# HeewoongNoh/DOSTransformer

Measured on NVIDIA B200. Metric: train-step crystals/sec (fwd+bwd), higher is better.
Workload: dtype bf16x3 operands, f32 accumulate

## Files before the change

dostransformer_b200/_lib.py:

```python
from __future__ import annotations

import ctypes as C
import os
from typing import Optional

import torch

_HERE = os.path.dirname(os.path.abspath(__file__))
LIB_PATH = os.environ.get("DOST_B200_LIB") or os.path.join(_HERE, "libdost_b200.so")

F32, F64 = 0, 1
ACT_NONE, ACT_RELU, ACT_LEAKY, ACT_PRELU = 0, 1, 2, 3
KC, MC = 0, 1
PREC_FMA, PREC_BF16X3, PREC_BF16 = 0, 1, 2
PRECISIONS = {"fp32": PREC_FMA, "bf16x3": PREC_BF16X3, "bf16": PREC_BF16}

_lib: Optional[C.CDLL] = None
ABI_VERSION = 15
DEVERR_MESSAGES = {1: "an index (edge_index / batch / system) is outside its table",
                   2: "a crystal has more atoms than the padding length given by the host (max_num_nodes)"}


class Seg(C.Structure):
    _fields_ = [("base", C.c_void_p), ("ld", C.c_longlong), ("idx", C.c_void_p), ("div", C.c_int),
# ... 101 lines not shown
                                 C.c_void_p, C.c_longlong, C.c_void_p, C.c_void_p, C.c_int, C.c_int, C.c_int, C.c_int,
                                 C.c_double, C.c_double, C.c_ulonglong, C.c_void_p]),
    "dost_xattn_bwd_workspace_bytes": (C.c_size_t, [C.c_int, C.c_int, C.c_int, C.c_int]),
    "dost_xattn_bwd": (C.c_int, [C.c_int, C.c_void_p, C.c_void_p, C.c_longlong, C.c_void_p, C.c_void_p, C.c_void_p,
                                 C.c_void_p, C.c_void_p, C.c_void_p, C.c_void_p, C.c_longlong, C.c_void_p, C.c_void_p,
                                 C.c_void_p, C.c_void_p, C.c_int, C.c_int, C.c_int, C.c_int, C.c_longlong, C.c_double,
                                 C.c_double, C.c_ulonglong, C.c_void_p, C.c_size_t, C.c_void_p]),
    "dost_xattn_kv_ext_build": (C.c_int, [C.c_void_p, C.c_void_p, C.c_void_p, C.c_void_p, C.c_longlong, C.c_int, C.c_int, C.c_void_p,
                                          C.c_void_p, C.c_longlong, C.c_void_p]),
    "dost_xattn_kv_ext_split": (C.c_int, [C.c_void_p, C.c_void_p, C.c_void_p, C.c_longlong, C.c_int, C.c_int, C.c_void_p, C.c_void_p,
                                          C.c_void_p]),
    "dost_xattn_kv_pad_split": (C.c_int, [C.c_void_p, C.c_int, C.c_int, C.c_void_p, C.c_void_p, C.c_longlong, C.c_int, C.c_int, C.c_void_p,
                                          C.c_void_p, C.c_void_p]),
    "dost_xattn_softmax_fwd": (C.c_int, [C.c_void_p, C.c_void_p, C.c_void_p, C.c_longlong, C.c_int, C.c_int, C.c_int, C.c_double,
                                         C.c_void_p, C.c_void_p, C.c_longlong, C.c_void_p, C.c_double, C.c_ulonglong, C.c_void_p]),
    "dost_xattn_softmax_bwd": (C.c_int, [C.c_void_p, C.c_void_p, C.c_void_p, C.c_void_p, C.c_void_p, C.c_longlong, C.c_int, C.c_int,
                                         C.c_int, C.c_double, C.c_void_p, C.c_void_p, C.c_longlong, C.c_double, C.c_ulonglong,
                                         C.c_void_p]),
    "dost_softmax_fwd": (C.c_int, [C.c_int, C.c_void_p, C.c_void_p, C.c_void_p, C.c_longlong, C.c_int, C.c_longlong, C.c_double,
                                   C.c_double, C.c_ulonglong, C.c_void_p]),
    "dost_softmax_bwd": (C.c_int, [C.c_int, C.c_void_p, C.c_void_p, C.c_void_p, C.c_longlong, C.c_int, C.c_longlong, C.c_double,
                                   C.c_double, C.c_ulonglong, C.c_void_p]),
    "dost_softmax_fwd_planes": (C.c_int, [C.c_void_p, C.c_void_p, C.c_void_p, C.c_longlong, C.c_int, C.c_longlong, C.c_double,
                                          C.c_double, C.c_ulonglong, C.c_void_p, C.c_void_p, C.c_longlong, C.c_void_p]),
    "dost_softmax_bwd_planes": (C.c_int, [C.c_void_p, C.c_void_p, C.c_void_p, C.c_longlong, C.c_int, C.c_longlong, C.c_double,
                                          C.c_double, C.c_ulonglong, C.c_void_p, C.c_void_p, C.c_longlong, C.c_void_p]),
    "dost_attn_fused_supported": (C.c_int, [C.c_int, C.c_int, C.c_int]),
    "dost_attn_fused_fwd": (C.c_int, [C.c_void_p, C.c_void_p, C.c_longlong, C.c_void_p, C.c_void_p, C.c_longlong, C.c_longlong,
                                      C.c_int, C.c_int, C.c_int, C.c_int, C.c_void_p, C.c_void_p, C.c_void_p, C.c_int, C.c_double,
                                      C.c_void_p, C.c_longlong, C.c_void_p, C.c_void_p, C.c_void_p, C.c_longlong, C.c_int,
                                      C.c_double, C.c_ulonglong, C.c_void_p, C.c_void_p]),
    "dost_softmax_bwd_from_planes": (C.c_int, [C.c_void_p, C.c_void_p, C.c_longlong, C.c_void_p, C.c_longlong, C.c_longlong, C.c_int,
                                               C.c_double, C.c_void_p, C.c_void_p, C.c_longlong, C.c_void_p]),
    "dost_eval_metrics": (C.c_int, [C.c_int, C.c_void_p, C.c_void_p, C.c_int, C.c_int, C.c_int, C.c_void_p, C.c_void_p, C.c_void_p]),
    "dost_adamw_step": (C.c_int, [C.c_int, C.c_void_p, C.c_void_p, C.c_void_p, C.c_void_p, C.c_void_p, C.c_double, C.c_double,
                                  C.c_double, C.c_double, C.c_double, C.c_longlong, C.c_void_p]),
    "dost_loss_fwd": (C.c_int, [C.c_int, C.c_int, C.c_void_p, C.c_void_p, C.c_void_p, C.c_double, C.c_int, C.c_int,
                                C.c_void_p, C.c_void_p, C.c_void_p]),
    "dost_loss_bwd": (C.c_int, [C.c_int, C.c_int, C.c_void_p, C.c_void_p, C.c_void_p, C.c_double, C.c_int, C.c_int,
                                C.c_void_p, C.c_void_p, C.c_void_p, C.c_void_p, C.c_void_p]),
    "dost_collate_ptr": (C.c_int, [C.c_void_p, C.c_longlong, C.c_void_p, C.c_void_p, C.c_longlong, C.c_void_p, C.c_void_p,
                                   C.c_void_p, C.c_void_p, C.c_void_p]),
    "dost_collate_rows": (C.c_int, [C.c_void_p, C.c_void_p, C.c_void_p, C.c_void_p, C.c_longlong, C.c_longlong,
                                    C.c_longlong, C.c_void_p, C.c_void_p]),
    "dost_collate_index": (C.c_int, [C.c_void_p, C.c_longlong, C.c_void_p, C.c_void_p, C.c_void_p, C.c_void_p, C.c_void_p,
                                     C.c_longlong, C.c_longlong, C.c_longlong, C.c_void_p, C.c_void_p, C.c_void_p]),
    "dost_neighbor_count": (C.c_int, [C.c_void_p, C.c_void_p, C.c_void_p, C.c_void_p, C.c_longlong, C.c_double, C.c_int,
                                      C.c_void_p, C.c_void_p]),
    "dost_neighbor_fill": (C.c_int, [C.c_void_p, C.c_void_p, C.c_void_p, C.c_void_p, C.c_longlong, C.c_double, C.c_int,
                                     C.c_void_p, C.c_int, C.c_void_p, C.c_void_p, C.c_void_p, C.c_void_p, C.c_void_p,
                                     C.c_void_p]),
    "dost_knn_select": (C.c_int, [C.c_void_p, C.c_void_p, C.c_void_p, C.c_longlong, C.c_int, C.c_longlong, C.c_double,
                                  C.c_void_p, C.c_void_p, C.c_void_p, C.c_void_p]),
    "dost_gaussian_expand": (C.c_int, [C.c_void_p, C.c_longlong, C.c_double, C.c_double, C.c_int, C.c_double, C.c_void_p,
                                       C.c_void_p]),
}


def _with_seed_offset(args):
    i = args.index(C.c_ulonglong) + 1
    return args[:i] + [C.c_void_p] + args[i:]


for _name in ("dost_xattn_fwd", "dost_xattn_bwd", "dost_xattn_softmax_fwd", "dost_xattn_softmax_bwd", "dost_softmax_fwd",
              "dost_softmax_bwd", "dost_softmax_fwd_planes", "dost_softmax_bwd_planes", "dost_attn_fused_fwd"):
    _res, _args = _SIGNATURES[_name]
# ... 105 lines not shown
```

dostransformer_b200/csrc/tc_ptx.cuh:

```cuda
#pragma once
#include <cuda.h>
#include <cuda_bf16.h>
#include <cstdint>

namespace dost {
namespace ptx {

__device__ __forceinline__ uint32_t smem_u32(const void* p) { return static_cast<uint32_t>(__cvta_generic_to_shared(p)); }
__device__ __forceinline__ void mbar_init(uint32_t bar, uint32_t count) {
  asm volatile("mbarrier.init.shared::cta.b64 [%0], %1;" ::"r"(bar), "r"(count) : "memory");
}
__device__ __forceinline__ void mbar_arrive(uint32_t bar) {
  asm volatile("mbarrier.arrive.shared::cta.b64 _, [%0];" ::"r"(bar) : "memory");
}
__device__ __forceinline__ void mbar_expect_tx(uint32_t bar, uint32_t bytes) {
  asm volatile("mbarrier.arrive.expect_tx.shared::cta.b64 _, [%0], %1;" ::"r"(bar), "r"(bytes) : "memory");
}
__device__ __forceinline__ void mbar_wait(uint32_t bar, uint32_t parity) {
  asm volatile(
      "{\n\t"
      ".reg .pred P1;\n\t"
      "WAIT_LOOP:\n\t"
      "mbarrier.try_wait.parity.shared::cta.b64 P1, [%0], %1, %2;\n\t"
      "@P1 bra WAIT_DONE;\n\t"
// ... 47 lines not shown
}
__device__ __forceinline__ uint32_t cluster_ctarank() {
  uint32_t r;
  asm volatile("mov.u32 %0, %%cluster_ctarank;" : "=r"(r));
  return r;
}
__device__ __forceinline__ void cluster_sync_all() {
  asm volatile("barrier.cluster.arrive.release.aligned;" ::: "memory");
  asm volatile("barrier.cluster.wait.acquire.aligned;" ::: "memory");
}
__device__ __forceinline__ uint32_t mapa_rank(uint32_t addr, uint32_t rank) {
  uint32_t r;
  asm volatile("mapa.shared::cluster.u32 %0, %1, %2;" : "=r"(r) : "r"(addr), "r"(rank));
  return r;
}
__device__ __forceinline__ void mbar_arrive_cluster(uint32_t cluster_bar) {
  asm volatile("mbarrier.arrive.relaxed.cluster.shared::cluster.b64 _, [%0];" ::"r"(cluster_bar) : "memory");
}
__device__ __forceinline__ void umma_commit_2cta(uint32_t bar) {
  asm volatile("tcgen05.commit.cta_group::2.mbarrier::arrive::one.shared::cluster.multicast::cluster.b64 [%0], %1;" ::"r"(bar),
               "h"(static_cast<uint16_t>(3))
               : "memory");
}
__device__ __forceinline__ void umma_f16_2cta(uint32_t tmem_d, uint64_t adesc, uint64_t bdesc, uint32_t idesc, uint32_t accum) {
  asm volatile(
      "{\n\t"
      ".reg .pred p;\n\t"
      "setp.ne.b32 p, %4, 0;\n\t"
      "tcgen05.mma.cta_group::2.kind::f16 [%0], %1, %2, %3, p;\n\t"
      "}" ::"r"(tmem_d),
      "l"(adesc), "l"(bdesc), "r"(idesc), "r"(accum)
      : "memory");
}
__device__ __forceinline__ void tma_load_3d_2cta(uint32_t dst, const CUtensorMap* map, int c0, int c1, int c2, uint32_t cluster_bar) {
  asm volatile(
      "cp.async.bulk.tensor.3d.cta_group::2.shared::cluster.global.mbarrier::complete_tx::bytes [%0], [%1, {%2, %3, %4}], [%5];" ::"r"(
          dst),
      "l"(map), "r"(c0), "r"(c1), "r"(c2), "r"(cluster_bar)
      : "memory");
}

__device__ __forceinline__ void tmem_ld_wait() { asm volatile("tcgen05.wait::ld.sync.aligned;" ::: "memory"); }

__device__ __forceinline__ void tma_load_3d(uint32_t dst, const CUtensorMap* map, int c0, int c1, int c2, uint32_t bar) {
  asm volatile(
      "cp.async.bulk.tensor.3d.shared::cluster.global.mbarrier::complete_tx::bytes [%0], [%1, {%2, %3, %4}], [%5];" ::"r"(dst),
      "l"(map), "r"(c0), "r"(c1), "r"(c2), "r"(bar)
      : "memory");
}

__device__ __forceinline__ uint32_t make_idesc(int m, int n, bool a_mn, bool b_mn) {
  return (1u << 4) | (1u << 7) | (1u << 10) | ((a_mn ? 1u : 0u) << 15) | ((b_mn ? 1u : 0u) << 16) |
         (static_cast<uint32_t>(n >> 3) << 17) | (static_cast<uint32_t>(m >> 4) << 24);
}

__device__ __forceinline__ void sts128(uint32_t addr, uint32_t a, uint32_t b, uint32_t c, uint32_t d) {
  asm volatile("st.shared.v4.b32 [%0], {%1, %2, %3, %4};" ::"r"(addr), "r"(a), "r"(b), "r"(c), "r"(d) : "memory");
}
__device__ __forceinline__ float4 lds128(uint32_t addr) {
  float4 v;
  asm volatile("ld.shared.v4.f32 {%0, %1, %2, %3}, [%4];" : "=f"(v.x), "=f"(v.y), "=f"(v.z), "=f"(v.w) : "r"(addr) : "memory");
  return v;
}


__device__ __forceinline__ void tma_store_3d(const CUtensorMap* map, uint32_t src, int c0, int c1, int c2) {
// ... 43 lines not shown
```

dostransformer_b200/ops.py:

```python
from __future__ import annotations

import ctypes as C
import math
from contextlib import nullcontext
import os
from dataclasses import dataclass, field
from typing import List, Optional, Sequence, Tuple

import torch

from . import _lib as L

NUM_SMS = 148

_PRECISION = L.PREC_FMA


def set_precision(name: str) -> None:
    global _PRECISION
    _PRECISION = L.PRECISIONS[name]


def get_precision() -> int:
    return _PRECISION
# ... 402 lines not shown
    if residual is not None:
        g.residual, g.ld_res = residual.data_ptr(), (ld_res if ld_res is not None else _ld(residual))
    if out is not None:
        g.out = out.data_ptr()
        g.ldc = ldc if ldc is not None else _ld(out)
    g.accumulate = 1 if accumulate else 0
    g.batch, g.a_bstride, g.b_bstride, g.c_bstride, g.res_bstride = batch, a_bstride, b_bstride, c_bstride, res_bstride
    g.b_rowoff = b_rowoff.data_ptr() if b_rowoff is not None else None
    g.c_rowoff = c_rowoff.data_ptr() if c_rowoff is not None else None
    g.c_rowlim = c_rowlim.data_ptr() if c_rowlim is not None else None
    if out_planes is not None:
        g.out_hi = out_planes.hi.data_ptr()
        g.out_lo = out_planes.lo.data_ptr() if out_planes.lo is not None else None
        g.ld_op = out_planes.ld
    g.split_k = split_k
    g.precision = _PRECISION if prec is None else prec
    g.colsum = colsum_out.data_ptr() if colsum_out is not None else None
    if out_gate is not None:
        g.out_gate, g.ld_gate = out_gate.data_ptr(), out_gate.stride(0)
    if dact_gate is not None:
        g.dact_gate, g.ld_gate, g.dact_slope = dact_gate.data_ptr(), dact_gate.stride(0), dact_slope
    lib = L.lib()
    ws, nb = None, 0
    if split_k > 1 or colsum_out is not None:
        nb = lib.dost_gemm_bf16_workspace_bytes(C.byref(g))
        ws = _ws(nb, b.hi.device)
    L.check(lib.dost_gemm_bf16(C.byref(g), L.p(ws), nb, L.stream()), "gemm_bf16")


def gate_bits_ok(M: int, N: int) -> bool:
    return M >= 32 and N % 32 == 0 and os.environ.get("DOST_GEMM_TMA_EPI", "1") != "0" and not L.switch("DOST_NO_FFN_GATE")


def tc_active(t: torch.Tensor) -> bool:
    return _PRECISION != L.PREC_FMA and t.dtype == torch.float32


def _with_lo() -> bool:
    return _PRECISION != L.PREC_BF16


def ln_fwd_planes(x2d: torch.Tensor, gamma, beta, slope=None, *, want_y: bool = False, want_planes: bool = True,
                  gather_add=None):
    M, W = x2d.shape
    ga = ia = gb = ib = None
    ldg = 0
    if gather_add is not None:
        ga, ia, gb, ib = gather_add
        ldg = _ld(ga)
        assert _ld(gb) == ldg
    dev = x2d.device
    y = torch.empty(M, W, dtype=torch.float32, device=dev) if want_y else None
    pl = empty_planes(M, W, dev, _with_lo()) if want_planes else None
    stats = torch.empty(M, 2, dtype=torch.float32, device=dev)
    L.check(L.lib().dost_ln_fwd_planes(L.p(x2d), _ld(x2d), L.p(ga), L.p(ia), L.p(gb), L.p(ib), ldg, L.p(gamma), L.p(beta),
                                       L.p(slope), L.p(y),
                                       L.p(pl.hi) if pl else None, L.p(pl.lo) if (pl and pl.lo is not None) else None,
                                       pl.ld if pl else 0, L.p(stats), M, W, L.stream()), "ln_fwd_planes")
    return y, pl, stats


def ln_bwd_planes(dy2d, x2d, stats, gamma, beta, slope=None, *, dres=None, want_dx: bool = True, want_planes: bool = False,
                  want_xsum: bool = False):
    M, W = x2d.shape
    dev = x2d.device
    dx = torch.empty(M, W, dtype=torch.float32, device=dev) if want_dx else None
# ... 21 lines not shown
    L.check(lib.dost_colsum_planes(L.p(pl.hi), L.p(pl.lo), pl.ld, pl.rows, pl.cols, L.p(out), L.p(ws), nb, L.stream()),
            "colsum_planes")
    return out


def _split_for(M_out: int, N_out: int, K_red: int) -> int:
    bn = 64 if N_out <= 64 else (128 if N_out <= 128 else 256)
    tiles = math.ceil(M_out / 128) * math.ceil(N_out / bn)
    want = max(1, (2 * NUM_SMS) // tiles)
    return int(max(1, min(want, math.ceil(K_red / 512), 256)))


def _planes_save(pl: Planes):
    return [pl.hi, pl.lo]


def _planes_load(hi, lo, rows, cols) -> Planes:
    return Planes(hi, lo, rows, cols)


class _FFNBlock(torch.autograd.Function):

    @staticmethod
    def forward(ctx, y_nd, ln_w, ln_b, w1, b1, w2, b2):
        H = y_nd.shape[-1]
        y = y_nd.reshape(-1, H)
        if y.stride(-1) != 1 or (y.shape[0] > 1 and y.stride(0) != H):
            y = y.contiguous()
        M = y.shape[0]
        F = w1.shape[0]
        dev = y.device
        _, h0p, stats = ln_fwd_planes(y, ln_w, ln_b)
        w1p, w2p = weight_planes(w1), weight_planes(w2)
        h1p = empty_planes(M, F, dev, _with_lo())
        gate = torch.empty(F // 32, M, dtype=torch.int32, device=dev) if (gate_bits_ok(M, F) and any(ctx.needs_input_grad)) else None
        gemm_planes(M=M, N=F, K=H, a=[h0p], a_mode=L.KC, b=w1p, b_mode=L.KC, bias=b1, act=L.ACT_RELU, out_planes=h1p, out_gate=gate)
        out = torch.empty(M, H, dtype=torch.float32, device=dev)
        gemm_planes(M=M, N=H, K=F, a=[h1p], a_mode=L.KC, b=w2p, b_mode=L.KC, bias=b2, residual=y, out=out)
        ctx.save_for_backward(y, stats, ln_w, ln_b, w1, w2, *_planes_save(h0p), *_planes_save(h1p), gate)
        ctx.prec = _PRECISION
        ctx.shape = y_nd.shape
        ctx.emit_grad_planes = bool(getattr(y_nd, "_dost_attn_out", False))
        return out.view(y_nd.shape)

    @staticmethod
    def backward(ctx, d_out_nd):
        y, stats, ln_w, ln_b, w1, w2, h0h, h0l, h1h, h1l, gate = ctx.saved_tensors
        M, H = y.shape
        F = w1.shape[0]
        dev = y.device
        with precision_value(ctx.prec):
            h0p, h1p = _planes_load(h0h, h0l, M, H), _planes_load(h1h, h1l, M, F)
            w1p, w2p = weight_planes(w1), weight_planes(w2)
            dop = getattr(d_out_nd, "_dost_planes", None)
            db2 = getattr(d_out_nd, "_dost_colsum", None)
            d_out = d_out_nd.reshape(M, H)
            if d_out.stride(-1) != 1 or (M > 1 and d_out.stride(0) != H):
                d_out, dop = d_out.contiguous(), None
            if dop is None or db2 is None or dop.rows != M or dop.cols != H or (dop.lo is not None) != _with_lo() or \
                    getattr(d_out_nd, "_dost_planes_version", -1) != d_out_nd._version:
                dop, db2 = split_planes_colsum(d_out)
            dw2 = torch.empty(H, F, dtype=torch.float32, device=dev)
            gemm_planes(M=H, N=F, K=M, a=[dop], a_mode=L.MC, b=h1p, b_mode=L.MC, out=dw2, split_k=_split_for(H, F, M))
            dv1p = empty_planes(M, F, dev, _with_lo())
            db1 = torch.empty(F, dtype=torch.float32, device=dev)
            gemm_planes(M=M, N=F, K=H, a=[dop], a_mode=L.KC, b=w2p, b_mode=L.MC, dact=h1p if gate is None else None,
                        dact_gate=gate, dact_slope=0.0, out_planes=dv1p, colsum_out=db1)
            dw1 = torch.empty(F, H, dtype=torch.float32, device=dev)
            gemm_planes(M=F, N=H, K=M, a=[dv1p], a_mode=L.MC, b=h0p, b_mode=L.MC, out=dw1, split_k=_split_for(F, H, M))
            dh0 = torch.empty(M, H, dtype=torch.float32, device=dev)
            gemm_planes(M=M, N=H, K=F, a=[dv1p], a_mode=L.KC, b=w1p, b_mode=L.MC, out=dh0)
            dy, dyp, dg, db, _, _ = ln_bwd_planes(dh0, y, stats, ln_w, ln_b, dres=d_out, want_planes=ctx.emit_grad_planes)
# ... 1059 lines not shown
```

include/dost.h:

```cpp
#ifndef DOST_H_
#define DOST_H_

#include <stddef.h>
#include <stdint.h>

#ifdef __cplusplus
extern "C" {
#endif

#define DOST_ABI_VERSION 15

enum { DOST_F32 = 0, DOST_F64 = 1 };
enum { DOST_OK = 0, DOST_ERR_ARG = -1, DOST_ERR_LAUNCH = -2, DOST_ERR_WORKSPACE = -3, DOST_ERR_UNSUPPORTED = -4 };
enum { DOST_ACT_NONE = 0, DOST_ACT_RELU = 1, DOST_ACT_LEAKY = 2, DOST_ACT_PRELU = 3 };
enum { DOST_PREC_FMA = 0, DOST_PREC_BF16X3 = 1 , DOST_PREC_BF16 = 2 };
enum { DOST_KC = 0 , DOST_MC = 1  };

typedef void* dost_stream_t;

int dost_abi_version(void);
const char* dost_last_error(void);
long long dost_launch_count(void);
void dost_reset_launch_count(void);

// ... 179 lines not shown
                     double drop_p, unsigned long long seed, dost_stream_t stream);
int dost_softmax_fwd_dseed(int dtype, const void* s, void* p, void* pd, long long rows, int cols, long long ld, double scale,
                           double drop_p, unsigned long long seed, const unsigned long long* seed_offset, dost_stream_t stream);
int dost_softmax_bwd_dseed(int dtype, const void* p, const void* dpd, void* ds, long long rows, int cols, long long ld,
                           double scale, double drop_p, unsigned long long seed, const unsigned long long* seed_offset,
                           dost_stream_t stream);

int dost_softmax_fwd_planes(const float* s, float* p, float* pd, long long rows, int cols, long long ld, double scale,
                            double drop_p, unsigned long long seed, void* hi, void* lo, long long ldp, dost_stream_t stream);
int dost_softmax_bwd_planes(const float* p, const float* dpd, float* ds, long long rows, int cols, long long ld, double scale,
                            double drop_p, unsigned long long seed, void* hi, void* lo, long long ldp, dost_stream_t stream);
int dost_softmax_fwd_planes_dseed(const float* s, float* p, float* pd, long long rows, int cols, long long ld, double scale,
                                  double drop_p, unsigned long long seed, const unsigned long long* seed_offset, void* hi,
                                  void* lo, long long ldp, dost_stream_t stream);
int dost_softmax_bwd_planes_dseed(const float* p, const float* dpd, float* ds, long long rows, int cols, long long ld,
                                  double scale, double drop_p, unsigned long long seed, const unsigned long long* seed_offset,
                                  void* hi, void* lo, long long ldp, dost_stream_t stream);

int dost_attn_fused_supported(int Lq, int H, int max_keys);
int dost_attn_fused_fwd(const void* q_hi, const void* q_lo, long long ld_q, const void* k_hi, const void* k_lo, long long ld_k,
                        long long k_rows, int S, int Lq, int Lk, int H, const int32_t* k_rowoff, const int32_t* k_count,
                        const int32_t* nmax, int max_keys, double scale, const float* residual, long long res_seq_stride,
                        float* out, void* p_hi, void* p_lo, long long ld_p, int precision, double drop_p,
                        unsigned long long seed, float* lse, dost_stream_t stream);
int dost_attn_fused_fwd_dseed(const void* q_hi, const void* q_lo, long long ld_q, const void* k_hi, const void* k_lo,
                              long long ld_k, long long k_rows, int S, int Lq, int Lk, int H, const int32_t* k_rowoff,
                              const int32_t* k_count, const int32_t* nmax, int max_keys, double scale, const float* residual,
                              long long res_seq_stride, float* out, void* p_hi, void* p_lo, long long ld_p, int precision,
                              double drop_p, unsigned long long seed, const unsigned long long* seed_offset, float* lse,
                              dost_stream_t stream);
int dost_softmax_bwd_from_planes(const void* p_hi, const void* p_lo, long long ld_pp, const float* dP, long long ld_dp,
                                 long long rows, int cols, double scale, void* hi, void* lo, long long ldp, dost_stream_t stream);

int dost_loss_fwd(int dtype, int mode, const void* pred_g, const void* pred_s, const void* y, double beta, int B,
                  int T, void* loss, void* saved, dost_stream_t stream);
int dost_loss_bwd(int dtype, int mode, const void* pred_g, const void* pred_s, const void* y, double beta, int B,
                  int T, const void* saved, const void* grad_loss, void* d_pred_g, void* d_pred_s,
                  dost_stream_t stream);

int dost_eval_metrics(int dtype, const void* pred, const void* y, int clamp_pred, int B, int T, void* per_crystal, void* mean,
                      dost_stream_t stream);

int dost_adamw_step(int ntensors, void* const* params, const void* const* grads, void* const* exp_avg,
                    void* const* exp_avg_sq, const long long* numel, double lr, double beta1, double beta2, double eps,
                    double weight_decay, long long step, dost_stream_t stream);

int dost_collate_ptr(const int64_t* ids, long long B, const int64_t* node_ptr_all, const int64_t* edge_ptr_all,
                     long long C, int64_t* node_ptr_out, int64_t* edge_ptr_out, int64_t* nmax_out, int32_t* bad_flag,
                     dost_stream_t stream);
int dost_collate_rows(const void* src, const int64_t* src_ptr_all, const int64_t* ids, const int64_t* out_ptr,
                      long long B, long long rows_out, long long row_bytes, void* dst, dost_stream_t stream);
int dost_collate_index(const int64_t* edge_index_all, long long E_all, const int64_t* node_ptr_all,
                       const int64_t* edge_ptr_all, const int64_t* ids, const int64_t* node_ptr_out,
                       const int64_t* edge_ptr_out, long long B, long long N_out, long long E_out,
                       int64_t* edge_index_out, int64_t* batch_out, dost_stream_t stream);

int dost_neighbor_count(const double* lattice, const double* pos, const int64_t* node_ptr, const int64_t* crystal_of,
                        long long N, double cutoff, int self_interaction, int64_t* count, dost_stream_t stream);
int dost_neighbor_fill(const double* lattice, const double* pos, const int64_t* node_ptr, const int64_t* crystal_of,
                       long long N, double cutoff, int self_interaction, const int64_t* edge_ptr, int local_ids,
                       int64_t* edge_src, int64_t* edge_dst, int64_t* edge_shift, double* edge_vec, double* edge_len,
                       dost_stream_t stream);
int dost_knn_select(const int64_t* edge_ptr, const int64_t* edge_dst, const double* edge_len, long long N, int k,
                    long long pad_idx, double pad_dist, int64_t* out_idx, double* out_dist, int64_t* out_edge,
                    dost_stream_t stream);
int dost_gaussian_expand(const double* dist, long long n, double dmin, double step, int nfilt, double var, float* out,
// ... 7 lines not shown
```

Measured before the change: 21090.

## Fuse FFN forward into a single 2-CTA tcgen05 kernel keeping hidden in TMEM

```diff
diff --git a/dostransformer_b200/_lib.py b/dostransformer_b200/_lib.py
--- a/dostransformer_b200/_lib.py
+++ b/dostransformer_b200/_lib.py
@@ -157,6 +157,11 @@
                                       C.c_double, C.c_ulonglong, C.c_void_p, C.c_void_p]),
     "dost_softmax_bwd_from_planes": (C.c_int, [C.c_void_p, C.c_void_p, C.c_longlong, C.c_void_p, C.c_longlong, C.c_longlong, C.c_int,
                                                C.c_double, C.c_void_p, C.c_void_p, C.c_longlong, C.c_void_p]),
+    "dost_ffn_fused_supported": (C.c_int, [C.c_int, C.c_int, C.c_int]),
+    "dost_ffn_fwd_fused": (C.c_int, [C.c_int, C.c_int, C.c_int, C.c_int, C.c_void_p, C.c_void_p, C.c_longlong, C.c_void_p,
+                                     C.c_void_p, C.c_longlong, C.c_void_p, C.c_void_p, C.c_void_p, C.c_longlong, C.c_void_p,
+                                     C.c_void_p, C.c_longlong, C.c_void_p, C.c_longlong, C.c_void_p, C.c_void_p, C.c_longlong,
+                                     C.c_void_p, C.c_longlong, C.c_void_p]),
     "dost_eval_metrics": (C.c_int, [C.c_int, C.c_void_p, C.c_void_p, C.c_int, C.c_int, C.c_int, C.c_void_p, C.c_void_p, C.c_void_p]),
     "dost_adamw_step": (C.c_int, [C.c_int, C.c_void_p, C.c_void_p, C.c_void_p, C.c_void_p, C.c_void_p, C.c_double, C.c_double,
                                   C.c_double, C.c_double, C.c_double, C.c_longlong, C.c_void_p]),
diff --git a/dostransformer_b200/csrc/ffn_fused.cu b/dostransformer_b200/csrc/ffn_fused.cu
--- /dev/null
+++ b/dostransformer_b200/csrc/ffn_fused.cu
@@ -0,0 +1,491 @@
+#include <cuda.h>
+#include <cuda_bf16.h>
+#include "common.cuh"
+#include "tc_ptx.cuh"
+
+namespace dost {
+namespace ffn {
+
+using namespace ptx;
+
+__device__ __forceinline__ void mbar_arrive_release_cluster(uint32_t cluster_bar) {
+  asm volatile("mbarrier.arrive.release.cluster.shared::cluster.b64 _, [%0];" ::"r"(cluster_bar) : "memory");
+}
+
+constexpr int BM = 128, BK = 64, FC = 128, HD = 256;
+constexpr int kEpiWarps = 8, kThreads = (kEpiWarps + 2) * 32;
+constexpr int kStgBytes = 4096;
+constexpr int kStageRing = 192 * 1024;
+constexpr int kSmemBytes = kStageRing + kEpiWarps * kStgBytes + 1024;
+constexpr int kMaxStages = 8;
+
+struct Maps {
+  CUtensorMap x_hi, x_lo, w1_hi, w1_lo, w2_hi, w2_lo;
+  CUtensorMap out, h_hi, h_lo;
+};
+
+struct Params {
+  int M, F, m_tiles;
+  const float* b1;
+  const float* b2;
+  const float* res; long long ld_res;
+  unsigned int* gate; long long ld_gate;
+  int store_h;
+};
+
+template <int NSPLIT>
+__global__ void __launch_bounds__(kThreads, 1) ffn_fwd_kernel(const __grid_constant__ Maps maps, const Params p) {
+  constexpr bool SPLIT = NSPLIT == 3;
+  constexpr int NP = SPLIT ? 2 : 1;
+  constexpr int XB = BM * BK * 2;
+  constexpr int W1B = (FC / 2) * BK * 2;
+  constexpr int W2B = (HD / 2) * BK * 2;
+  constexpr int A_BYTES = NP * (XB + W1B), B_BYTES = NP * W2B;
+  constexpr int STAGE = A_BYTES;
+  constexpr int NSTAGE = kStageRing / STAGE;
+  static_assert(B_BYTES <= STAGE && NSTAGE >= 2 && NSTAGE <= kMaxStages, "stage ring");
+
+  extern __shared__ __align__(1024) unsigned char smem_raw[];
+  unsigned char* smem = reinterpret_cast<unsigned char*>((reinterpret_cast<uintptr_t>(smem_raw) + 1023) & ~uintptr_t(1023));
+  __shared__ __align__(8) unsigned long long bars[2 * kMaxStages + 6];
+  __shared__ uint32_t tmem_base_s;
+
+  const int warp = threadIdx.x >> 5, lane = threadIdx.x & 31;
+  const uint32_t full0 = smem_u32(&bars[0]), empty0 = smem_u32(&bars[kMaxStages]);
+  const uint32_t acc1f0 = smem_u32(&bars[2 * kMaxStages]);
+  const uint32_t pready0 = smem_u32(&bars[2 * kMaxStages + 2]);
+  const uint32_t acc2f = smem_u32(&bars[2 * kMaxStages + 4]);
+  const uint32_t acc2e = smem_u32(&bars[2 * kMaxStages + 5]);
+  const int NC = p.F / FC;
+  const int rank = (int)cluster_ctarank();
+  const int tile0 = (int)(blockIdx.x >> 1), tile_step = (int)(gridDim.x >> 1);
+
+  if (threadIdx.x == 0) {
+    for (int s = 0; s < NSTAGE; ++s) {
+      mbar_init(full0 + 8 * s, 1);
+      mbar_init(empty0 + 8 * s, 1);
+    }
+    for (int b = 0; b < 2; ++b) {
+      mbar_init(acc1f0 + 8 * b, 1);
+      mbar_init(pready0 + 8 * b, 2 * kEpiWarps);
+    }
+    mbar_init(acc2f, 1);
+    mbar_init(acc2e, 2 * kEpiWarps);
+    fence_barrier_init();
+  }
+  if (warp == kEpiWarps) {
+    asm volatile("tcgen05.alloc.cta_group::2.sync.aligned.shared::cta.b32 [%0], %1;" ::"r"(smem_u32(&tmem_base_s)), "r"(512) : "memory");
+    asm volatile("tcgen05.relinquish_alloc_permit.cta_group::2.sync.aligned;" ::: "memory");
+  }
+  tc_fence_before();
+  __syncthreads();
+  cluster_sync_all();
+  tc_fence_after();
+  const uint32_t tmem_base = tmem_base_s;
+
+  if (warp == kEpiWarps + 1) {
+    if (lane == 0) {
+      int stage = 0;
+      uint32_t phase = 0;
+      auto next = [&]() {
+        if (++stage == NSTAGE) {
+          stage = 0;
+          phase ^= 1;
+        }
+      };
+      for (int tile = tile0; tile < p.m_tiles; tile += tile_step) {
+        const int m0 = tile * 2 * BM + rank * BM;
+        auto begin = [&](int bytes) {
+          mbar_wait(empty0 + 8 * stage, phase ^ 1);
+          if (rank == 0) mbar_expect_tx(full0 + 8 * stage, 2 * bytes);
+          return mapa_rank(full0 + 8 * stage, 0);
+        };
+        auto load_a = [&](int c) {
+          for (int kt = 0; kt < HD / BK; ++kt) {
+            const uint32_t bar = begin(A_BYTES);
+            const uint32_t s = smem_u32(smem + stage * STAGE);
+            const int w1row = c * FC + rank * (FC / 2);
+            tma_load_3d_2cta(s, &maps.x_hi, kt * BK, m0, 0, bar);
+            tma_load_3d_2cta(s + NP * XB, &maps.w1_hi, kt * BK, w1row, 0, bar);
+            if (SPLIT) {
+              tma_load_3d_2cta(s + XB, &maps.x_lo, kt * BK, m0, 0, bar);
+              tma_load_3d_2cta(s + 2 * XB + W1B, &maps.w1_lo, kt * BK, w1row, 0, bar);
+            }
+            next();
+          }
+        };
+        auto load_b = [&](int c) {
+          for (int kt = 0; kt < FC / BK; ++kt) {
+            const uint32_t bar = begin(B_BYTES);
+            const uint32_t s = smem_u32(smem + stage * STAGE);
+            tma_load_3d_2cta(s, &maps.w2_hi, c * FC + kt * BK, rank * (HD / 2), 0, bar);
+            if (SPLIT) tma_load_3d_2cta(s + W2B, &maps.w2_lo, c * FC + kt * BK, rank * (HD / 2), 0, bar);
+            next();
+          }
+        };
+        load_a(0);
+        for (int c = 1; c < NC; ++c) {
+          load_a(c);
+          load_b(c - 1);
+        }
+        load_b(NC - 1);
+      }
+    }
+  } else if (warp == kEpiWarps) {
+    const uint32_t idesc1 = make_idesc(2 * BM, FC, false, false), idesc2 = make_idesc(2 * BM, HD, false, false);
+    int stage = 0;
+    uint32_t phase = 0;
+    auto next = [&]() {
+      if (++stage == NSTAGE) {
+        stage = 0;
+        phase ^= 1;
+      }
+    };
+    int g = 0;
+    int local = 0;
+    for (int tile = tile0; tile < p.m_tiles && rank == 0; tile += tile_step, ++local) {
+      auto issue_a = [&](int gc) {
+        const uint32_t tmem_d = tmem_base + (gc & 1) * FC;
+        for (int kt = 0; kt < HD / BK; ++kt) {
+          mbar_wait(full0 + 8 * stage, phase);
+          tc_fence_after();
+          if (lane == 0) {
+            const uint32_t s = smem_u32(smem + stage * STAGE);
+            const uint64_t dxh = make_smem_desc(s, 0), dwh = make_smem_desc(s + NP * XB, 0);
+            const uint64_t dxl = make_smem_desc(s + XB, 0), dwl = make_smem_desc(s + 2 * XB + W1B, 0);
+#pragma unroll
+            for (int ks = 0; ks < BK / 16; ++ks) {
+              const uint64_t adv = static_cast<uint64_t>(ks * (32 >> 4));
+              const uint32_t first = (kt > 0 || ks > 0) ? 1u : 0u;
+              if (SPLIT) {
+                umma_f16_2cta(tmem_d, dxl + adv, dwh + adv, idesc1, first);
+                umma_f16_2cta(tmem_d, dxh + adv, dwl + adv, idesc1, 1u);
+                umma_f16_2cta(tmem_d, dxh + adv, dwh + adv, idesc1, 1u);
+              } else {
+                umma_f16_2cta(tmem_d, dxh + adv, dwh + adv, idesc1, first);
+              }
+            }
+            umma_commit_2cta(empty0 + 8 * stage);
+            if (kt == HD / BK - 1) umma_commit_2cta(acc1f0 + 8 * (gc & 1));
+          }
+          __syncwarp();
+          next();
+        }
+      };
+      auto issue_b = [&](int c, int gc) {
+        mbar_wait(pready0 + 8 * (gc & 1), (gc >> 1) & 1);
+        if (c == 0) mbar_wait(acc2e, (local & 1) ^ 1);
+        tc_fence_after();
+        const uint32_t tmem_a = tmem_base + (gc & 1) * FC;
+        for (int kt = 0; kt < FC / BK; ++kt) {
+          mbar_wait(full0 + 8 * stage, phase);
+          tc_fence_after();
+          if (lane == 0) {
+            const uint32_t s = smem_u32(smem + stage * STAGE);
+            const uint64_t dwh = make_smem_desc(s, 0), dwl = make_smem_desc(s + W2B, 0);
+#pragma unroll
+            for (int ks = 0; ks < BK / 16; ++ks) {
+              const int kstep = kt * (BK / 16) + ks;
+              const uint64_t adv = static_cast<uint64_t>(ks * (32 >> 4));
+              const uint32_t ah = tmem_a + 16 * kstep;
+              const uint32_t acc = (c > 0 || kstep > 0) ? 1u : 0u;
+              if (SPLIT) {
+                umma_f16_ts_2cta(tmem_base + 2 * FC, ah + 8, dwh + adv, idesc2, acc);
+                umma_f16_ts_2cta(tmem_base + 2 * FC, ah, dwl + adv, idesc2, 1u);
+                umma_f16_ts_2cta(tmem_base + 2 * FC, ah, dwh + adv, idesc2, 1u);
+              } else {
+                umma_f16_ts_2cta(tmem_base + 2 * FC, ah, dwh + adv, idesc2, acc);
+              }
+            }
+            umma_commit_2cta(empty0 + 8 * stage);
+            if (c == NC - 1 && kt == FC / BK - 1) umma_commit_2cta(acc2f);
+          }
+          __syncwarp();
+          next();
+        }
+      };
+      issue_a(g);
+      for (int c = 1; c < NC; ++c) {
+        issue_a(g + c);
+        issue_b(c - 1, g + c - 1);
+      }
+      issue_b(NC - 1, g + NC - 1);
+      g += NC;
+    }
+  } else {
+    const int quad = warp & 3, half = warp >> 2;
+    const uint32_t stg = smem_u32(smem + kStageRing) + warp * kStgBytes;
+    const uint32_t lane_off = static_cast<uint32_t>(quad * 32) << 16;
+    const uint32_t pready_l0 = mapa_rank(pready0, 0), acc2e_l = mapa_rank(acc2e, 0);
+    const bool store_h = p.store_h != 0;
+    int g = 0;
+    int local = 0;
+    for (int tile = tile0; tile < p.m_tiles; tile += tile_step, ++local) {
+      const int mw = tile * 2 * BM + rank * BM + quad * 32;
+      const int mrow = mw + lane;
+      const bool row_ok = mrow < p.M;
+      for (int c = 0; c < NC; ++c, ++g) {
+        const int buf = g & 1;
+        float4 bq[8];
+        const float* bp = p.b1 + c * FC + half * 64;
+#pragma unroll
+        for (int j = 0; j < 8; ++j) bq[j] = __ldg(reinterpret_cast<const float4*>(bp) + j);
+        mbar_wait(acc1f0 + 8 * buf, (g >> 1) & 1);
+        tc_fence_after();
+#pragma unroll 1
+        for (int sub = 0; sub < 2; ++sub) {
+          const int col = half * 64 + sub * 32;
+          const int n0 = c * FC + col;
+          const uint32_t taddr = tmem_base + lane_off + buf * FC + col;
+          uint32_t r[32];
+          tmem_ld32(taddr, r);
+          tmem_ld_wait();
+          float v[32];
+#pragma unroll
+          for (int j = 0; j < 32; ++j) v[j] = __uint_as_float(r[j]);
+          if (sub == 1) {
+#pragma unroll
+            for (int j = 0; j < 8; ++j) bq[j] = __ldg(reinterpret_cast<const float4*>(bp + 32) + j);
+          }
+#pragma unroll
+          for (int j = 0; j < 8; ++j) {
+            v[4 * j] += bq[j].x; v[4 * j + 1] += bq[j].y; v[4 * j + 2] += bq[j].z; v[4 * j + 3] += bq[j].w;
+          }
+          uint32_t bits = 0u;
+#pragma unroll
+          for (int j = 0; j < 32; ++j) bits |= (v[j] > 0.f ? 1u : 0u) << j;
+          const float slope = 0.f;
+#pragma unroll
+          for (int j = 0; j < 32; ++j) v[j] = (v[j] > 0.f) ? v[j] : slope * v[j];
+          uint32_t hi[16], lo[16];
+#pragma unroll
+          for (int j = 0; j < 16; ++j) {
+            hi[j] = pack_bf16(v[2 * j], v[2 * j + 1]);
+            lo[j] = pack_bf16(v[2 * j] - __uint_as_float(hi[j] << 16), v[2 * j + 1] - __uint_as_float(hi[j] & 0xFFFF0000u));
+          }
+          uint32_t t[32];
+#pragma unroll
+          for (int j = 0; j < 8; ++j) {
+            t[j] = hi[j]; t[8 + j] = lo[j]; t[16 + j] = hi[8 + j]; t[24 + j] = lo[8 + j];
+          }
+          tmem_st32(taddr, t);
+          if (store_h) {
+            if (row_ok) p.gate[(long long)(n0 >> 5) * p.ld_gate + mrow] = bits;
+            if (lane == 0) bulk_wait_read0();
+            __syncwarp();
+            const uint32_t sw = (lane >> 1) & 3;
+#pragma unroll
+            for (int q = 0; q < 4; ++q) {
+              sts128(stg + lane * 64 + ((q ^ sw) << 4), hi[4 * q], hi[4 * q + 1], hi[4 * q + 2], hi[4 * q + 3]);
+              if (SPLIT) sts128(stg + 2048 + lane * 64 + ((q ^ sw) << 4), lo[4 * q], lo[4 * q + 1], lo[4 * q + 2], lo[4 * q + 3]);
+            }
+            fence_async_smem();
+            __syncwarp();
+            if (lane == 0 && mw < p.M) {
+              tma_store_3d(&maps.h_hi, stg, n0, mw, 0);
+              if (SPLIT) tma_store_3d(&maps.h_lo, stg + 2048, n0, mw, 0);
+              bulk_commit();
+            }
+          }
+        }
+        tmem_st_wait();
+        tc_fence_before();
+        __syncwarp();
+        if (lane == 0) mbar_arrive_release_cluster(pready_l0 + 8 * buf);
+      }
+      const float* rp = p.res + (long long)mrow * p.ld_res + half * 128;
+      uint4 rq[8];
+#pragma unroll
+      for (int j = 0; j < 8; ++j) rq[j] = row_ok ? __ldg(reinterpret_cast<const uint4*>(rp) + j) : make_uint4(0u, 0u, 0u, 0u);
+      mbar_wait(acc2f, local & 1);
+      tc_fence_after();
+#pragma unroll 1
+      for (int sub = 0; sub < 4; ++sub) {
+        const int n0 = half * 128 + sub * 32;
+        uint32_t r[32];
+        tmem_ld32(tmem_base + lane_off + 2 * FC + n0, r);
+        tmem_ld_wait();
+        if (sub == 3) {
+          tc_fence_before();
+          __syncwarp();
+          if (lane == 0) mbar_arrive_cluster(acc2e_l);
+        }
+        float v[32];
+#pragma unroll
+        for (int j = 0; j < 8; ++j) {
+          const float4 b = __ldg(reinterpret_cast<const float4*>(p.b2 + n0) + j);
+          v[4 * j] = __uint_as_float(r[4 * j]) + b.x;
+          v[4 * j + 1] = __uint_as_float(r[4 * j + 1]) + b.y;
+          v[4 * j + 2] = __uint_as_float(r[4 * j + 2]) + b.z;
+          v[4 * j + 3] = __uint_as_float(r[4 * j + 3]) + b.w;
+        }
+#pragma unroll
+        for (int j = 0; j < 8; ++j) {
+          v[4 * j] += __uint_as_float(rq[j].x); v[4 * j + 1] += __uint_as_float(rq[j].y);
+          v[4 * j + 2] += __uint_as_float(rq[j].z); v[4 * j + 3] += __uint_as_float(rq[j].w);
+        }
+        if (sub < 3) {
+#pragma unroll
+          for (int j = 0; j < 8; ++j)
+            rq[j] = row_ok ? __ldg(reinterpret_cast<const uint4*>(rp + 32 * (sub + 1)) + j) : make_uint4(0u, 0u, 0u, 0u);
+        }
+        if (lane == 0) bulk_wait_read0();
+        __syncwarp();
+#pragma unroll
+        for (int j = 0; j < 8; ++j)
+          sts128(stg + lane * 128 + ((j ^ (lane & 7)) << 4), __float_as_uint(v[4 * j]), __float_as_uint(v[4 * j + 1]),
+                 __float_as_uint(v[4 * j + 2]), __float_as_uint(v[4 * j + 3]));
+        fence_async_smem();
+        __syncwarp();
+        if (lane == 0 && mw < p.M) {
+          tma_store_3d(&maps.out, stg, n0, mw, 0);
+          bulk_commit();
+        }
+      }
+    }
+    if (lane == 0) bulk_wait0();
+  }
+
+  tc_fence_before();
+  __syncthreads();
+  cluster_sync_all();
+  if (warp == kEpiWarps) {
+    tc_fence_after();
+    asm volatile("tcgen05.dealloc.cta_group::2.sync.aligned.b32 %0, %1;" ::"r"(tmem_base), "r"(512) : "memory");
+  }
+}
+
+typedef CUresult (*EncodeTiledFn)(CUtensorMap*, CUtensorMapDataType, cuuint32_t, void*, const cuuint64_t*, const cuuint64_t*,
+                                  const cuuint32_t*, const cuuint32_t*, CUtensorMapInterleave, CUtensorMapSwizzle,
+                                  CUtensorMapL2promotion, CUtensorMapFloatOOBfill);
+
+static EncodeTiledFn encode_fn() {
+  static EncodeTiledFn fn = [] {
+    void* ptr = nullptr;
+    cudaDriverEntryPointQueryResult q;
+    if (cudaGetDriverEntryPoint("cuTensorMapEncodeTiled", &ptr, cudaEnableDefault, &q) != cudaSuccess || q != cudaDriverEntryPointSuccess)
+      ptr = nullptr;
+    return reinterpret_cast<EncodeTiledFn>(ptr);
+  }();
+  return fn;
+}
+
+static int make_map(CUtensorMap* m, const void* base, bool f32, long long inner, long long rows, long long ld, int box_inner,
+                    int box_rows, CUtensorMapSwizzle swz, CUtensorMapL2promotion l2) {
+  EncodeTiledFn fn = encode_fn();
+  if (!fn) {
+    set_error("ffn_fused: cuTensorMapEncodeTiled is not available");
+    return DOST_ERR_UNSUPPORTED;
+  }
+  const int esz = f32 ? 4 : 2;
+  cuuint64_t dims[3] = {(cuuint64_t)inner, (cuuint64_t)rows, 1};
+  cuuint64_t strides[2] = {(cuuint64_t)ld * esz, (cuuint64_t)(ld * rows * esz)};
+  cuuint32_t box[3] = {(cuuint32_t)box_inner, (cuuint32_t)box_rows, 1u};
+  cuuint32_t estr[3] = {1u, 1u, 1u};
+  CUresult r = fn(m, f32 ? CU_TENSOR_MAP_DATA_TYPE_FLOAT32 : CU_TENSOR_MAP_DATA_TYPE_BFLOAT16, 3, const_cast<void*>(base), dims,
+                  strides, box, estr, CU_TENSOR_MAP_INTERLEAVE_NONE, swz, l2, CU_TENSOR_MAP_FLOAT_OOB_FILL_NONE);
+  if (r != CUDA_SUCCESS) {
+    set_error("ffn_fused: cuTensorMapEncodeTiled failed (%d) base=%p inner=%lld rows=%lld ld=%lld", (int)r, base, inner, rows, ld);
+    return DOST_ERR_ARG;
+  }
+  return DOST_OK;
+}
+
+template <int NSPLIT>
+static int launch(const Maps& maps, const Params& p, cudaStream_t st) {
+  auto kern = ffn_fwd_kernel<NSPLIT>;
+  static PerDevice cfg_once;
+  if (bool* flag = cfg_once.pending()) {
+    cudaError_t e = cudaFuncSetAttribute(kern, cudaFuncAttributeMaxDynamicSharedMemorySize, kSmemBytes);
+    if (e != cudaSuccess) {
+      set_error("ffn_fused: cudaFuncSetAttribute failed: %s", cudaGetErrorString(e));
+      return DOST_ERR_LAUNCH;
+    }
+    *flag = true;
+  }
+  const int half_sms = sm_count() / 2;
+  const int pairs = p.m_tiles < half_sms ? p.m_tiles : half_sms;
+  cudaLaunchConfig_t cfg = {};
+  cfg.gridDim = dim3(2 * pairs);
+  cfg.blockDim = dim3(kThreads);
+  cfg.dynamicSmemBytes = kSmemBytes;
+  cfg.stream = st;
+  cudaLaunchAttribute attr[1];
+  attr[0].id = cudaLaunchAttributeClusterDimension;
+  attr[0].val.clusterDim.x = 2;
+  attr[0].val.clusterDim.y = 1;
+  attr[0].val.clusterDim.z = 1;
+  cfg.attrs = attr;
+  cfg.numAttrs = 1;
+  cudaError_t e = cudaLaunchKernelEx(&cfg, kern, maps, p);
+  if (e != cudaSuccess) {
+    set_error("ffn_fused: cluster launch failed: %s", cudaGetErrorString(e));
+    return DOST_ERR_LAUNCH;
+  }
+  return check_launch("ffn_fwd_fused");
+}
+
+static inline bool al16(const void* ptr) { return (reinterpret_cast<uintptr_t>(ptr) & 15) == 0; }
+
+}
+}
+
+using namespace dost;
+
+extern "C" int dost_ffn_fused_supported(int M, int H, int F) {
+  return (M >= 32 && H == ffn::HD && F >= ffn::FC && F % ffn::FC == 0) ? 1 : 0;
+}
+
+extern "C" int dost_ffn_fwd_fused(int M, int H, int F, int precision, const void* x_hi, const void* x_lo, long long ld_x,
+                                  const void* w1_hi, const void* w1_lo, long long ld_w1, const float* b1, const void* w2_hi,
+                                  const void* w2_lo, long long ld_w2, const float* b2, const float* residual, long long ld_res,
+                                  float* out, long long ld_out, void* h_hi, void* h_lo, long long ld_h, unsigned int* gate,
+                                  long long ld_gate, dost_stream_t stream) {
+  using namespace dost::ffn;
+  DOST_REQUIRE(dost_ffn_fused_supported(M, H, F), "ffn_fwd_fused: unsupported shape M=%d H=%d F=%d", M, H, F);
+  DOST_REQUIRE(precision == DOST_PREC_BF16X3 || precision == DOST_PREC_BF16, "ffn_fwd_fused: precision must be bf16x3 or bf16");
+  const bool split3 = precision == DOST_PREC_BF16X3;
+  DOST_REQUIRE(x_hi && w1_hi && w2_hi && b1 && b2 && residual && out, "ffn_fwd_fused: null pointer");
+  DOST_REQUIRE(!split3 || (x_lo && w1_lo && w2_lo), "ffn_fwd_fused: bf16x3 needs the lo planes");
+  DOST_REQUIRE(al16(x_hi) && al16(x_lo) && al16(w1_hi) && al16(w1_lo) && al16(w2_hi) && al16(w2_lo) && ld_x % 8 == 0 &&
+                   ld_w1 % 8 == 0 && ld_w2 % 8 == 0 && ld_x >= H && ld_w1 >= H && ld_w2 >= F,
+               "ffn_fwd_fused: operand planes must be 16-byte aligned with ld %% 8 == 0");
+  DOST_REQUIRE(al16(b1) && al16(b2) && al16(residual) && al16(out) && ld_res % 4 == 0 && ld_out % 4 == 0 && ld_res >= H && ld_out >= H,
+               "ffn_fwd_fused: bias / residual / out must be 16-byte aligned with ld %% 4 == 0");
+  const bool store_h = h_hi != nullptr;
+  DOST_REQUIRE(!store_h || (gate && (!split3 || h_lo) && al16(h_hi) && al16(h_lo) && ld_h % 8 == 0 && ld_h >= F && ld_gate >= M),
+               "ffn_fwd_fused: the hidden planes need gates, 16-byte alignment, ld %% 8 == 0 and ld_gate >= M");
+  Maps maps;
+  Params p;
+  p.M = M;
+  p.F = F;
+  p.m_tiles = (M + 2 * BM - 1) / (2 * BM);
+  p.b1 = b1;
+  p.b2 = b2;
+  p.res = residual;
+  p.ld_res = ld_res;
+  p.gate = gate;
+  p.ld_gate = ld_gate;
+  p.store_h = store_h ? 1 : 0;
+  const auto SW128 = CU_TENSOR_MAP_SWIZZLE_128B, SW64 = CU_TENSOR_MAP_SWIZZLE_64B;
+  const auto L2P = CU_TENSOR_MAP_L2_PROMOTION_L2_256B, L2N = CU_TENSOR_MAP_L2_PROMOTION_NONE;
+  int rc = ffn::make_map(&maps.x_hi, x_hi, false, H, M, ld_x, BK, BM, SW128, L2P);
+  if (rc == DOST_OK) rc = ffn::make_map(&maps.w1_hi, w1_hi, false, H, F, ld_w1, BK, FC / 2, SW128, L2P);
+  if (rc == DOST_OK) rc = ffn::make_map(&maps.w2_hi, w2_hi, false, F, H, ld_w2, BK, HD / 2, SW128, L2P);
+  if (rc == DOST_OK && split3) rc = ffn::make_map(&maps.x_lo, x_lo, false, H, M, ld_x, BK, BM, SW128, L2P);
+  if (rc == DOST_OK && split3) rc = ffn::make_map(&maps.w1_lo, w1_lo, false, H, F, ld_w1, BK, FC / 2, SW128, L2P);
+  if (rc == DOST_OK && split3) rc = ffn::make_map(&maps.w2_lo, w2_lo, false, F, H, ld_w2, BK, HD / 2, SW128, L2P);
+  if (rc == DOST_OK) rc = ffn::make_map(&maps.out, out, true, H, M, ld_out, 32, 32, SW128, L2N);
+  if (rc == DOST_OK && store_h) rc = ffn::make_map(&maps.h_hi, h_hi, false, F, M, ld_h, 32, 32, SW64, L2N);
+  if (rc == DOST_OK && store_h && split3) rc = ffn::make_map(&maps.h_lo, h_lo, false, F, M, ld_h, 32, 32, SW64, L2N);
+  if (rc != DOST_OK) return rc;
+  if (!split3) {
+    maps.x_lo = maps.x_hi;
+    maps.w1_lo = maps.w1_hi;
+    maps.w2_lo = maps.w2_hi;
+  }
+  if (!store_h) maps.h_hi = maps.out;
+  if (!store_h || !split3) maps.h_lo = maps.h_hi;
+  cudaStream_t st = (cudaStream_t)stream;
+  return split3 ? launch<3>(maps, p, st) : launch<1>(maps, p, st);
+}
diff --git a/dostransformer_b200/csrc/tc_ptx.cuh b/dostransformer_b200/csrc/tc_ptx.cuh
--- a/dostransformer_b200/csrc/tc_ptx.cuh
+++ b/dostransformer_b200/csrc/tc_ptx.cuh
@@ -103,6 +103,16 @@
       "l"(adesc), "l"(bdesc), "r"(idesc), "r"(accum)
       : "memory");
 }
+__device__ __forceinline__ void umma_f16_ts_2cta(uint32_t tmem_d, uint32_t tmem_a, uint64_t bdesc, uint32_t idesc, uint32_t accum) {
+  asm volatile(
+      "{\n\t"
+      ".reg .pred p;\n\t"
+      "setp.ne.b32 p, %4, 0;\n\t"
+      "tcgen05.mma.cta_group::2.kind::f16 [%0], [%1], %2, %3, p;\n\t"
+      "}" ::"r"(tmem_d),
+      "r"(tmem_a), "l"(bdesc), "r"(idesc), "r"(accum)
+      : "memory");
+}
 __device__ __forceinline__ void tma_load_3d_2cta(uint32_t dst, const CUtensorMap* map, int c0, int c1, int c2, uint32_t cluster_bar) {
   asm volatile(
       "cp.async.bulk.tensor.3d.cta_group::2.shared::cluster.global.mbarrier::complete_tx::bytes [%0], [%1, {%2, %3, %4}], [%5];" ::"r"(
diff --git a/dostransformer_b200/ops.py b/dostransformer_b200/ops.py
--- a/dostransformer_b200/ops.py
+++ b/dostransformer_b200/ops.py
@@ -458,6 +458,10 @@
     return M >= 32 and N % 32 == 0 and os.environ.get("DOST_GEMM_TMA_EPI", "1") != "0" and not L.switch("DOST_NO_FFN_GATE")
 
 
+def ffn_fused_ok(M: int, H: int, F: int) -> bool:
+    return gate_bits_ok(M, F) and not L.switch("DOST_NO_FFN_FUSED") and L.lib().dost_ffn_fused_supported(M, H, F) == 1
+
+
 def tc_active(t: torch.Tensor) -> bool:
     return _PRECISION != L.PREC_FMA and t.dtype == torch.float32
 
@@ -545,12 +549,24 @@
         dev = y.device
         _, h0p, stats = ln_fwd_planes(y, ln_w, ln_b)
         w1p, w2p = weight_planes(w1), weight_planes(w2)
-        h1p = empty_planes(M, F, dev, _with_lo())
-        gate = torch.empty(F // 32, M, dtype=torch.int32, device=dev) if (gate_bits_ok(M, F) and any(ctx.needs_input_grad)) else None
-        gemm_planes(M=M, N=F, K=H, a=[h0p], a_mode=L.KC, b=w1p, b_mode=L.KC, bias=b1, act=L.ACT_RELU, out_planes=h1p, out_gate=gate)
+        training = any(ctx.needs_input_grad)
         out = torch.empty(M, H, dtype=torch.float32, device=dev)
-        gemm_planes(M=M, N=H, K=F, a=[h1p], a_mode=L.KC, b=w2p, b_mode=L.KC, bias=b2, residual=y, out=out)
-        ctx.save_for_backward(y, stats, ln_w, ln_b, w1, w2, *_planes_save(h0p), *_planes_save(h1p), gate)
+        if ffn_fused_ok(M, H, F):
+            h1p = empty_planes(M, F, dev, _with_lo()) if training else None
+            gate = torch.empty(F // 32, M, dtype=torch.int32, device=dev) if training else None
+            L.check(L.lib().dost_ffn_fwd_fused(
+                M, H, F, _PRECISION, L.p(h0p.hi), L.p(h0p.lo), h0p.ld, L.p(w1p.hi), L.p(w1p.lo), w1p.ld, L.p(b1),
+                L.p(w2p.hi), L.p(w2p.lo), w2p.ld, L.p(b2), L.p(y), _ld(y), L.p(out), _ld(out),
+                L.p(h1p.hi) if h1p else None, L.p(h1p.lo) if (h1p and h1p.lo is not None) else None, h1p.ld if h1p else 0,
+                L.p(gate), gate.stride(0) if gate is not None else 0, L.stream()), "ffn_fwd_fused")
+        else:
+            h1p = empty_planes(M, F, dev, _with_lo())
+            gate = torch.empty(F // 32, M, dtype=torch.int32, device=dev) if (gate_bits_ok(M, F) and training) else None
+            gemm_planes(M=M, N=F, K=H, a=[h0p], a_mode=L.KC, b=w1p, b_mode=L.KC, bias=b1, act=L.ACT_RELU, out_planes=h1p,
+                        out_gate=gate)
+            gemm_planes(M=M, N=H, K=F, a=[h1p], a_mode=L.KC, b=w2p, b_mode=L.KC, bias=b2, residual=y, out=out)
+        ctx.save_for_backward(y, stats, ln_w, ln_b, w1, w2, *_planes_save(h0p),
+                              *(_planes_save(h1p) if h1p is not None else [None, None]), gate)
         ctx.prec = _PRECISION
         ctx.shape = y_nd.shape
         ctx.emit_grad_planes = bool(getattr(y_nd, "_dost_attn_out", False))
diff --git a/include/dost.h b/include/dost.h
--- a/include/dost.h
+++ b/include/dost.h
@@ -235,6 +235,12 @@
 int dost_softmax_bwd_from_planes(const void* p_hi, const void* p_lo, long long ld_pp, const float* dP, long long ld_dp,
                                  long long rows, int cols, double scale, void* hi, void* lo, long long ldp, dost_stream_t stream);
 
+int dost_ffn_fused_supported(int M, int H, int F);
+int dost_ffn_fwd_fused(int M, int H, int F, int precision, const void* x_hi, const void* x_lo, long long ld_x, const void* w1_hi,
+                       const void* w1_lo, long long ld_w1, const float* b1, const void* w2_hi, const void* w2_lo, long long ld_w2,
+                       const float* b2, const float* residual, long long ld_res, float* out, long long ld_out, void* h_hi,
+                       void* h_lo, long long ld_h, unsigned int* gate, long long ld_gate, dost_stream_t stream);
+
 int dost_loss_fwd(int dtype, int mode, const void* pred_g, const void* pred_s, const void* y, double beta, int B,
                   int T, void* loss, void* saved, dost_stream_t stream);
 int dost_loss_bwd(int dtype, int mode, const void* pred_g, const void* pred_s, const void* y, double beta, int B,
```

After: 21260, median of 6. No clear change (+0.8%).
